# Ledicia/Molecular-Dynamics-Simulation---Lennard-Jones-monoatomic-fluid

Hardware: AMD Instinct MI355X
Metric: md_steps_per_sec_n262144_fp64 (higher is better)
Workload: dtype f64

## Files before the change

molecular-dynamics-simulation---lennard-jones-monoatomic-fluid_amd/csrc/ljmd_capi.cpp:

```cpp
#include "ljmd_engine.h"
#include "ljmd_multi.h"

#include <new>

namespace ljmdh {

int entry_checks(const ljmd_t *h, const char *who, unsigned checks)
{
    if ((checks & kHandle) && !h) return fail(nullptr, LJMD_ERR_INVALID_ARG, "%s: NULL handle", who);
    if ((checks & kHaveState) && !h->have_state) return fail(h, LJMD_ERR_STATE, "%s: no state has been set", who);
    if ((checks & kHaveAccel) && !h->have_accel)
        return fail(h, LJMD_ERR_STATE, "%s: accelerations not initialised (call ljmd_compute_forces first)", who);
    if ((checks & kNotPoisoned) && h->poisoned)
        return fail(h, LJMD_ERR_STATE, "%s: handle poisoned by an earlier failure; call ljmd_set_state", who);
    return LJMD_OK;
}

}

extern "C" {

const char *ljmd_version(void) { return "ljmd 0.6.0 gfx950"; }

int32_t ljmd_device_count(void)
// ... 61 lines not shown
                      int32_t n_gpus, const int32_t *devices)
{
    return ljmdm::create(out, n, box_length, dt, rc, precision_mode, n_gpus, devices);
}


int ljmd_set_state(ljmd_t *h, const double *rx, const double *ry, const double *rz,
                   const double *vx, const double *vy, const double *vz)
{
    LJMD_TRY(entry_checks(h, "ljmd_set_state", kHandle));
    if (!rx || !ry || !rz || !vx || !vy || !vz)
        return fail(h, LJMD_ERR_INVALID_ARG, "ljmd_set_state: NULL array");
    if (h->multi) return ljmdm::set_state(h, rx, ry, rz, vx, vy, vz);
    h->boxes_valid = false;
    h->drift_prefused = false;
    h->step_open = false;
    ljmdt::tcf_new_trajectory(&h->tcf);
    LJMD_HIP(h, hipSetDevice(h->device));
    if (h->poisoned) {
        LJMD_HIP(h, hipStreamSynchronize(h->stream));
        LJMD_HIP(h, hipMemcpy(&h->ring_issued, h->d_ring_pos, sizeof(unsigned), hipMemcpyDeviceToHost));
        h->ring_consumed = h->ring_issued;
        h->forces_pending = false;
        h->gather_done_for_step = false;
        h->fold_pending = false;
        h->poisoned = false;
    }
    const size_t S = h->plan.S, P = h->plan.P;
    double lo[3] = {INFINITY, INFINITY, INFINITY}, hi[3] = {-INFINITY, -INFINITY, -INFINITY};
    const double *src[3] = {rx, ry, rz};
    bool finite = true;
    for (int g = 0; g < h->G; ++g)
        for (int ax = 0; ax < 3; ++ax) {
            double *dst = h->h_stage + ((size_t)g * 3 + ax) * P;
            const double *s = src[ax] + (size_t)g * S;
// ... 123 lines not shown
{
    if (h->multi) return ljmdm::enqueue_steps(h, nsteps, sampled);
    static_assert(LJMD_MAX_PENDING_STEPS == kRingCap, "LJMD_MAX_PENDING_STEPS out of sync with the record ring");
    if (ring_guard && (h->ring_issued - h->ring_consumed) + (unsigned)nsteps > kRingCap)
        return fail(h, LJMD_ERR_STATE, "%s: %u + %d pending steps exceed LJMD_MAX_PENDING_STEPS", who,
                    h->ring_issued - h->ring_consumed, nsteps);
    LJMD_HIP(h, hipSetDevice(h->device));
    const bool keep = h->want_energy;
    for (int s = 0; s < nsteps; ++s) {
        EventSet *q = next_events(h);
        if (sampled) h->want_energy = s == nsteps - 1;
        int rc_ = enqueue_drift(h, q);
        if (rc_ == LJMD_OK) rc_ = enqueue_forces(h, true, q, s + 1 < nsteps);
        if (rc_ != LJMD_OK) {
            h->want_energy = keep;
            h->poisoned = true;
            return rc_;
        }
    }
    h->want_energy = keep;
    return LJMD_OK;
}

int collect_steps(ljmd_t *h, int32_t nsteps, double *epot, double *ekin, double *d_epot, double *dd_epot, const char *who)
{
    LJMD_TRY(entry_checks(h, who, kHandle));
    if (nsteps < 0 || nsteps > (int)kRingCap) return fail(h, LJMD_ERR_INVALID_ARG, "%s: nsteps out of range", who);
    LJMD_TRY(entry_checks(h, who, kNotPoisoned));
    if (h->multi) return ljmdm::collect_steps(h, nsteps, epot, ekin, d_epot, dd_epot);
    if (h->G != 1) return fail(h, LJMD_ERR_STATE, "%s: sharded engine; use ljmd_read_partials", who);
// ... 389 lines not shown
```

molecular-dynamics-simulation---lennard-jones-monoatomic-fluid_amd/csrc/ljmd_common.cpp:

```cpp
#include "ljmd_common.h"
#include "ljmd_internal.h"

#include <algorithm>
#include <cstdio>
#include <cstring>
#include <limits>

namespace ljmdh {

using namespace ljmdk;

thread_local std::string g_last_error = "";

int failv(std::string *handle_err, int code, const char *fmt, va_list ap)
{
    char buf[512];
    vsnprintf(buf, sizeof buf, fmt, ap);
    g_last_error = buf;
    if (handle_err) *handle_err = buf;
    return code;
}

int check_sim_params(const char *who, int n, double box_length, double dt, double rc)
{
// ... 50 lines not shown
        const char *v = std::getenv(name);
        if (v && *v) return std::atoi(v);
        return std::nullopt;
    };
    Knobs k;
    k.sort = flag("LJMD_SORT", k.sort);
    k.force_generic = flag("LJMD_FORCE_GENERIC", k.force_generic);
    k.force_collectives = flag("LJMD_FORCE_COLLECTIVES", k.force_collectives);
    k.fuse = flag("LJMD_FUSE", k.fuse);
    k.fuse_tail = flag("LJMD_FUSE_TAIL", k.fuse_tail);
    k.fuse_defer_record = flag("LJMD_FUSE_DEFER_RECORD", k.fuse_defer_record);
    k.xcd_remap = std::max(0, env_int("LJMD_N3_XCD_REMAP", k.xcd_remap));
    k.inject_failure_at_step = env_int("LJMD_INJECT_FAILURE_AT_STEP", k.inject_failure_at_step);
    k.exchange_alltoall = is("LJMD_FORCE_EXCHANGE", "alltoall");
    k.resort_every = opt_int("LJMD_RESORT_EVERY");
    k.n3_row_tiles = env_int("LJMD_N3_ROW_TILES", k.n3_row_tiles);
    k.n3_wg_waves = env_int("LJMD_N3_WG_WAVES", k.n3_wg_waves);
    k.slab_budget_gb = std::max(1, env_int("LJMD_SLAB_BUDGET_GB", k.slab_budget_gb));
    k.n3_both_ties = flag("LJMD_N3_BOTH_TIES", k.n3_both_ties);
    k.n3_min_n = env_int("LJMD_N3_MIN_N", k.n3_min_n);
    k.n3 = flag("LJMD_N3", k.n3);
    k.n3_target_waves = opt_int("LJMD_N3_TARGET_WAVES");
    k.n3_clusters = flag("LJMD_N3_CLUSTERS", k.n3_clusters);
    k.n3_pertile = flag("LJMD_N3_PERTILE", k.n3_pertile);
    k.reduce_split = opt_int("LJMD_REDUCE_SPLIT");
    if (k.reduce_split) k.reduce_split = std::max(0, *k.reduce_split);
    k.walk_chunk = opt_int("LJMD_WALK_CHUNK");
    k.fp32_far_stream = flag("LJMD_FP32_FAR_STREAM", k.fp32_far_stream);
    k.fp32_vfar = flag("LJMD_FP32_VFAR", k.fp32_vfar);
    {
// ... 87 lines not shown
```

molecular-dynamics-simulation---lennard-jones-monoatomic-fluid_amd/csrc/ljmd_common.h:

```cpp
#ifndef LJMD_COMMON_H
#define LJMD_COMMON_H

#include "ljmd.h"

#include <hip/hip_runtime.h>

#include <cstdarg>
#include <cstddef>
#include <cstdint>
#include <cstdlib>
#include <optional>
#include <string>

namespace ljmdh {

extern thread_local std::string g_last_error;

constexpr double kPi = 3.1415926535897932384626433832795;

int failv(std::string *handle_err, int code, const char *fmt, va_list ap);

inline int fail(std::nullptr_t, int code, const char *fmt, ...)
{
    va_list ap;
// ... 57 lines not shown

void scalars_from_exact_sums(const uint64_t (&ordered)[5][3], double te, double td, double tdd, bool have_e, bool have_k,
                             double *epot, double *ekin, double *d_epot, double *dd_epot);

struct Knobs {
    bool sort = true;
    bool force_generic = false;
    bool force_collectives = false;
    bool fuse = true;
    bool fuse_tail = true;
    bool fuse_defer_record = true;
    int xcd_remap = 4;
    int inject_failure_at_step = -1;
    bool exchange_alltoall = false;
    std::optional<int> resort_every;
    int n3_row_tiles = 0;
    int n3_wg_waves = 0;
    int slab_budget_gb = 64;
    bool n3_both_ties = true;
    int n3_min_n = 4096;
    bool n3 = true;
    std::optional<int> n3_target_waves;
    bool n3_clusters = true;
    bool n3_pertile = true;
    std::optional<int> reduce_split;
    std::optional<int> walk_chunk;
    bool fp32_far_stream = true;
    bool fp32_vfar = true;
    double fp32_split = 5.0;
    bool overlap_exchange = true;
// ... 11 lines not shown
```

molecular-dynamics-simulation---lennard-jones-monoatomic-fluid_amd/csrc/ljmd_engine.cpp:

```cpp
#include "ljmd_engine.h"

namespace ljmdh {

bool fast_path_ok(const ljmd_t *h) { return h->plan.rc_allows_fast && h->positions_compact && !h->knobs.force_generic; }

double *wg_part_now(ljmd_t *h) { return h->d_wg_part + (h->plan.fuse_tail ? (size_t)h->fold_parity * h->wg_part_stride : 0); }

PairArgs pair_args(ljmd_t *h, bool fast)
{
    PairArgs a;
    a.pos = h->d_pos;
    a.slab = h->d_slab;
    a.wg_part = wg_part_now(h);
    a.mask = h->d_mask;
    a.bbox = h->d_bbox;
    a.inline_mask = (fast && h->plan.fuse_tail && !h->plan.use_n3) ? 1 : 0;
    a.rc2_skin = h->rc2 * (1.0 + 1e-10);
    a.n = h->n;
    a.S = h->plan.S;
    a.P = h->plan.P;
    a.G = h->G;
    a.rank = h->rank;
    a.TB = h->plan.TB;
    a.T = h->plan.T;
// ... 133 lines not shown

EventSet *next_events(ljmd_t *h)
{
    if (!h->profiling || h->ev_used >= (size_t)kMaxProfiledLaunches) return nullptr;
    if (h->ev_used == h->ev_pool.size()) {
        EventSet q;
        for (auto &e : q.e)
            if (hipEventCreate(&e) != hipSuccess) return nullptr;
        h->ev_pool.push_back(q);
    }
    EventSet *q = &h->ev_pool[h->ev_used++];
    q->has_pos_x = q->has_force_x = false;
    return q;
}

int resort(ljmd_t *h, bool with_accel)
{
    {
    LJMD_HIP(h, launch_iota(h->d_idx, h->plan.P, h->stream));
    LJMD_HIP(h, hipMemcpyAsync(h->d_idx2, h->d_idx, (size_t)h->plan.P * sizeof(int), hipMemcpyDeviceToDevice,
                               h->stream));
    int *cur = h->d_idx, *nxt = h->d_idx2;
    for (size_t l = 0; l < h->plan.kd_level_nseg.size(); ++l) {
        const double *axis = own_block(h) + (size_t)h->kd_axis[l] * h->plan.P;
        LJMD_HIP(h, kd_level(h->d_cub, h->cub_bytes, axis, h->L, h->d_kd_keys, h->d_kd_keys2, cur, nxt, h->plan.S,
                             h->plan.kd_level_nseg[l], h->d_kd_offsets + h->plan.kd_level_off[l], h->stream));
        std::swap(cur, nxt);
    }
    if (cur != h->d_idx2)
        LJMD_HIP(h, hipMemcpyAsync(h->d_idx2, cur, (size_t)h->plan.P * sizeof(int), hipMemcpyDeviceToDevice,
                                   h->stream));
    }
    const size_t bytes3 = 3 * (size_t)h->plan.P * sizeof(double);
    double *sets[4] = {own_block(h), h->d_ru, h->d_v, h->d_a};
    for (int k = 0; k < (with_accel ? 4 : 3); ++k) {
        LJMD_HIP(h, launch_gather3(sets[k], h->d_tmp3, h->d_idx2, h->plan.P, h->stream));
        LJMD_HIP(h, hipMemcpyAsync(sets[k], h->d_tmp3, bytes3, hipMemcpyDeviceToDevice, h->stream));
    }
    LJMD_HIP(h, launch_gather_perm(h->d_perm, h->d_perm2, h->d_idx2, h->plan.P, h->stream));
    std::swap(h->d_perm, h->d_perm2);
    h->perm_dirty = true;
    h->steps_since_sort = 0;
    return LJMD_OK;
}

int refresh_perm(ljmd_t *h)
{
    if (!h->perm_dirty) return LJMD_OK;
    LJMD_HIP(h, hipMemcpyAsync(h->h_perm.data(), h->d_perm, (size_t)h->plan.P * sizeof(int), hipMemcpyDeviceToHost,
                               h->stream));
    LJMD_HIP(h, hipStreamSynchronize(h->stream));
    h->perm_dirty = false;
    return LJMD_OK;
}

bool use_comm_stream(const ljmd_t *h) { return h->knobs.overlap_exchange && h->comm_stream != nullptr; }

int comm_begin(ljmd_t *h)
// ... 65 lines not shown
                                          h->mode == LJMD_PRECISION_FP32_FORCE ? h->d_desc_far : nullptr, h->d_desc2, h->stream));
        else
            LJMD_HIP(h, launch_tile_mask(ga, h->stream));
        if (q) LJMD_HIP(h, hipEventRecord(q->e[2], h->stream));
        if (h->plan.use_n3) {
            const dim3 grid((h->plan.NGo + h->plan.wg_waves - 1) / h->plan.wg_waves, h->plan.nslab_n);
            N3Args na = n3_args(h);
            na.xcd_remap = (h->knobs.xcd_remap > 0 && (int)grid.x >= kXcdMinGroups && grid.x % (8 * h->knobs.xcd_remap) == 0) ? h->knobs.xcd_remap : 0;
            const bool far_beside = h->mode == LJMD_PRECISION_FP32_FORCE && h->far_stream != nullptr;
            split = h->plan.split_s1 > 0 && h->side_stream != nullptr;
            if (split) {
                const int s1 = h->plan.split_s1;
                LJMD_HIP(h, hipEventRecord(h->ev_side_go, h->stream));
                LJMD_HIP(h, hipStreamWaitEvent(h->side_stream, h->ev_side_go, 0));
                LJMD_HIP(h, launch_pair_n3(na, dim3(grid.x, s1), h->plan.wg_waves, h->stream));
                N3Args nb = na;
                nb.by0 = s1;
                LJMD_HIP(h, launch_pair_n3(nb, dim3(grid.x, grid.y - s1), h->plan.wg_waves, h->side_stream));
                LJMD_HIP(h, launch_reduce_forces_split(reduce_args(h, h->plan.nslab_n, true), 1, h->stream));
                LJMD_HIP(h, hipEventRecord(h->ev_side_done, h->side_stream));
                LJMD_HIP(h, hipStreamWaitEvent(h->stream, h->ev_side_done, 0));
            } else if (far_beside) {
                LJMD_HIP(h, hipEventRecord(h->ev_far_go, h->stream));
                LJMD_HIP(h, hipStreamWaitEvent(h->far_stream, h->ev_far_go, 0));
            } else {
                LJMD_HIP(h, launch_pair_n3(na, grid, h->plan.wg_waves, h->stream));
            }
            nslab = h->plan.nslab_n;
            n_wg = grid.x * grid.y * h->plan.wg_waves;
            n3 = true;
            if (h->mode == LJMD_PRECISION_FP32_FORCE) {
                const dim3 fgrid(h->plan.NGo, h->plan.nslab_n);
                N3Args fa = n3_args(h);
                fa.mask = h->d_mask_far;
                fa.slab_i = h->d_slab + (size_t)h->plan.nslab_n * 3 * h->plan.P;
                fa.slab_j = h->d_slab_j2;
// ... 163 lines not shown

int enqueue_drift_positions(ljmd_t *h, EventSet *q, bool *split)
{
    if (q) LJMD_HIP(h, hipEventRecord(q->e[0], h->stream));
    h->gather_done_for_step = false;
    const bool resort_now = h->plan.sort_enabled && fast_path_ok(h) && h->steps_since_sort + 1 >= h->plan.resort_every;
    *split = !resort_now;
    LJMD_HIP(h, launch_drift_kick(integrate_args(h), resort_now ? 0 : 1, h->stream));
    h->positions_compact = true;
    h->positions_wide = false;
    if (h->plan.sort_enabled && fast_path_ok(h) && ++h->steps_since_sort >= h->plan.resort_every) {
        if (*split) {
            LJMD_HIP(h, launch_drift_kick(integrate_args(h), 2, h->stream));
            *split = false;
        }
        return resort(h, false);
    }
    return LJMD_OK;
}

int enqueue_drift_velocities(ljmd_t *h)
{
    LJMD_HIP(h, launch_drift_kick(integrate_args(h), 2, h->stream));
    return LJMD_OK;
}

int enqueue_drift(ljmd_t *h, EventSet *q)
{
    const bool collectives = h->comm && (h->G > 1 || h->knobs.force_collectives);
    if (collectives && use_comm_stream(h)) {
        bool split = false;
// ... 11 lines not shown
        LJMD_HIP(h, hipEventRecord(h->ev_gather_done, h->comm_stream));
        rc_ = enqueue_drift_velocities(h);
        if (rc_ != LJMD_OK) return rc_;
        LJMD_HIP(h, hipStreamWaitEvent(h->stream, h->ev_gather_done, 0));
        h->gather_done_for_step = true;
        return LJMD_OK;
    }
    if (q) LJMD_HIP(h, hipEventRecord(q->e[0], h->stream));
    h->gather_done_for_step = false;
    const bool resort_now = h->plan.sort_enabled && fast_path_ok(h) && h->steps_since_sort + 1 >= h->plan.resort_every;
    if (h->drift_prefused) {
        h->drift_prefused = false;
        h->boxes_valid = !resort_now && fast_path_ok(h);
        h->positions_compact = true;
        h->positions_wide = false;
        if (h->plan.sort_enabled && fast_path_ok(h) && ++h->steps_since_sort >= h->plan.resort_every) return resort(h, false);
        return LJMD_OK;
    }
    IntegrateArgs ia = integrate_args(h);
    h->boxes_valid = h->knobs.fuse && h->G == 1 && h->n <= 65536 && !resort_now && fast_path_ok(h);
    if (h->boxes_valid) {
        ia.bbox = h->d_bbox;
        ia.pos_tc = h->plan.use_n3 ? h->d_pos_tc : nullptr;
    }
    LJMD_HIP(h, launch_drift_kick(ia, 0, h->stream));
    h->positions_compact = true;
    h->positions_wide = false;
    if (h->plan.sort_enabled && fast_path_ok(h) && ++h->steps_since_sort >= h->plan.resort_every)
        return resort(h, false);
    return LJMD_OK;
}

int fetch_ring(ljmd_t *h, unsigned count)
{
    if (count > h->ring_issued - h->ring_consumed)
        return fail(h, LJMD_ERR_STATE, "requested %u step records but only %u are pending", count,
                    h->ring_issued - h->ring_consumed);
    h->ring_consumed = h->ring_issued - count;
    unsigned done = 0;
    while (done < count) {
        const unsigned pos = (h->ring_consumed + done) % kRingCap;
        const unsigned run = std::min(count - done, kRingCap - pos);
        LJMD_HIP(h, hipMemcpyAsync(h->h_ring + (size_t)done * h->rec_stride,
                                   h->d_ring + (size_t)pos * h->rec_stride,
// ... 11 lines not shown
```

molecular-dynamics-simulation---lennard-jones-monoatomic-fluid_amd/csrc/ljmd_engine.h:

```cpp
#ifndef LJMD_ENGINE_H
#define LJMD_ENGINE_H

#include "ljmd_common.h"

#include <rccl/rccl.h>

#include <algorithm>
#include <cmath>
#include <cstdio>
#include <cstring>
#include <limits>
#include <mutex>
#include <vector>

#include "ljmd_internal.h"
#include "ljmd_resident.h"

using namespace ljmdk;

namespace ljmdh {

constexpr unsigned kRingCap = 4096;
constexpr int kTargetWorkgroups = 2048;
constexpr int kXcdMinGroups = 256;
constexpr int kMixedMinN = 16384;
constexpr long kN3ItemsFor4 = 6000;
constexpr long kN3ItemsFor2 = 1000;
constexpr long kN3LargeItems = 131072;
constexpr int kN3MidTargetItems = 32768;
constexpr int kBothTiesMaxGroups = 128;
constexpr int kFuseTailMaxRowTiles = 2;
constexpr int kFuseTailMaxN = 20000;
constexpr int kReduceSplitMinN = 131072;
constexpr int kReduceSplitShare = 8;
constexpr int kMaxProfiledLaunches = 4096;
constexpr int kEventsPerLaunch = 9;

struct EventSet {
    hipEvent_t e[kEventsPerLaunch];
    bool has_pos_x = false, has_force_x = false;
};

struct LaunchPlan {
    int S = 0, P = 0;
    int TB = 0, T = 0, W = 0;
    bool rc_allows_fast = false;
    bool sort_enabled = true;
    int resort_every = 20;
    std::vector<int> kd_level_nseg;
    std::vector<size_t> kd_level_off;
    std::vector<int> kd_offsets;
    int nslab_g = 1, chunk_g = 0;
    int nslab_t = 1, chunk_t = 0;
    bool use_n3 = false;
    int wg_waves = 1;
    bool both_ties = false;
    int uchunk = 0;
    int CS = 0, CS2 = 0, j_by_group = 0;
    int NG = 0, NGo = 0, Dmax = 0, nslab_n = 1, dchunk = 0;
    int rt = kRowTiles;
    bool fuse_tail = false;
    int split_s1 = 0, split_j1 = 0;
    int nslab_max = 1, n_wg_max = 0;
    int n_ke = 0;
};

int plan_engine(const SimParams &sim, int n, int n_ranks, int precision_mode, const Knobs &k, LaunchPlan *out);

}

struct ljmd_multi;

using namespace ljmdh;

struct ljmd : ljmdh::SimParams {
    ljmd_multi *multi = nullptr;
    bool poisoned = false;
// ... 48 lines not shown
    std::vector<int> kd_axis;
    int *d_kd_offsets = nullptr;
    unsigned long long *d_kd_keys = nullptr, *d_kd_keys2 = nullptr;

    unsigned ring_consumed = 0;
    unsigned ring_issued = 0;
    bool fold_pending = false;
    ljmdk::FinalizeArgs pending_fold{};
    int fold_parity = 0;
    size_t wg_part_stride = 0;
    double *d_slab_j = nullptr;
    unsigned char *d_flag_j = nullptr;
    double *d_red_part = nullptr;
    hipStream_t side_stream = nullptr;
    hipEvent_t ev_side_go = nullptr, ev_side_done = nullptr;
    uint64_t *d_mask_far = nullptr;
    double *d_slab_j2 = nullptr;
    unsigned char *d_flag_j2 = nullptr;
    double *d_fpart = nullptr, *d_frecv = nullptr;
    double *d_fall = nullptr;
    bool forces_pending = false;
    bool external_force_exchange = false;
    int pending_n_wg = 0;
    double pending_scale = 0.5;

    double *h_stage = nullptr;
    double *h_ring = nullptr;
    std::vector<int> h_perm;
    bool perm_dirty = false;

// ... 38 lines not shown

enum : unsigned { kHandle = 1, kHaveState = 2, kHaveAccel = 4, kNotPoisoned = 8 };
int entry_checks(const ljmd_t *h, const char *who, unsigned checks);

inline double *own_block(ljmd_t *h) { return h->d_pos + (size_t)h->rank * 3 * h->plan.P; }
inline bool needs_force_exchange(const ljmd_t *h) { return h->plan.use_n3 && (h->G > 1 || h->knobs.force_collectives); }
bool fast_path_ok(const ljmd_t *h);
IntegrateArgs integrate_args(ljmd_t *h);

int allocate_engine(ljmd_t *h);
void release(ljmd_t *h);
void release_resident(ljmd_t *h);
int download_state(ljmd_t *h, double *const dsts[12], unsigned n_records);
int upload_shard3(ljmd_t *h, double *dst, const double *x, const double *y, const double *z);
int resort(ljmd_t *h, bool with_accel);
int refresh_perm(ljmd_t *h);
bool use_comm_stream(const ljmd_t *h);
int comm_begin(ljmd_t *h);
int comm_end(ljmd_t *h);
int allgather_on(ljmd_t *h, hipStream_t s);

int enqueue_drift(ljmd_t *h, EventSet *q);
int enqueue_drift_positions(ljmd_t *h, EventSet *q, bool *split);
int enqueue_drift_velocities(ljmd_t *h);
int enqueue_pair_forces(ljmd_t *h, EventSet *q);
int enqueue_kick(ljmd_t *h, bool kick, EventSet *q);
int enqueue_forces(ljmd_t *h, bool kick, EventSet *q, bool next_drift = false);
int fetch_ring(ljmd_t *h, unsigned count);
void combine_one(const ljmd_t *h, const double *recs, int n_ranks, double *epot, double *ekin, double *d_epot,
                 double *dd_epot);
// ... 15 lines not shown
```

molecular-dynamics-simulation---lennard-jones-monoatomic-fluid_amd/csrc/ljmd_internal.h:

```cpp
#ifndef LJMD_INTERNAL_H
#define LJMD_INTERNAL_H

#include <hip/hip_runtime.h>
#include <stdint.h>

namespace ljmdk {

constexpr int kBlock = 256;
constexpr int kWavesPerBlock = kBlock / 64;
constexpr int kTile = 64;
#ifndef LJMD_ROW_TILES
#define LJMD_ROW_TILES 4
#endif
constexpr int kRowTiles = LJMD_ROW_TILES;
constexpr unsigned kAllRows = (1u << kRowTiles) - 1u;
constexpr int kSlotAlign = (kRowTiles * 64 > 256) ? kRowTiles * 64 : 256;
constexpr int kPartialStride = 8;
constexpr int kFoldBlocks = 128;
constexpr int kDirectFoldMax = 20480;
constexpr int kBoxStride = 8;

struct PairArgs {
    const double *pos;
    double *slab;
// ... 220 lines not shown
hipError_t launch_pair_fixed(const FixedArgs &a, dim3 grid, hipStream_t s);
hipError_t launch_fixed_tail(const FixedTailArgs &a, bool kick, bool energy, bool ke_only, hipStream_t s);
hipError_t launch_fixed_fold(const FixedFoldArgs &a, hipStream_t s);
hipError_t launch_rdf_histogram(const RdfArgs &a, dim3 grid, hipStream_t s);
hipError_t launch_time_origin(const TimeOriginArgs &a, bool vacf, int n_origins, hipStream_t s);
hipError_t launch_tile_boxes(const GeometryArgs &a, hipStream_t s);
hipError_t launch_tile_mask(const GeometryArgs &a, hipStream_t s);
hipError_t launch_tile_class(const GeometryArgs &a, double invL, double rc2, int S, int NGo, unsigned *desc,
                             unsigned *desc_far, float *desc2 , hipStream_t s);

size_t kd_temp_bytes(int count);
hipError_t launch_iota(int *idx, int P, hipStream_t s);
hipError_t kd_level(void *temp, size_t temp_bytes, const double *coord_axis, double L, unsigned long long *keys,
                    unsigned long long *keys_out, int *idx, int *idx_out, int S, int nseg, const int *seg_offsets,
                    hipStream_t s);
constexpr int kMigrateRows = 10;
hipError_t launch_iota_blocked(int *idx, int n, int S, int P, hipStream_t s);
hipError_t launch_iota_offset(int *idx, int count, int P, int offset, hipStream_t s);
hipError_t kd_level_blocked(void *temp, size_t temp_bytes, const double *pos, int axis, int P, double L,
                            unsigned long long *keys, unsigned long long *keys_out, int *idx, int *idx_out, int n, int nseg,
                            const int *seg_offsets, hipStream_t s);
hipError_t launch_migrate_pack(const double *ru, const double *v, const double *a, const int *perm, const int *gid0,
                               double *block, int S, int P, hipStream_t s);
hipError_t launch_migrate_select(const double *pos_all, const double *mig_all, const int *mine, double *new_pos, double *ru,
                                 double *v, double *a, int *gid0, int S, int P, hipStream_t s);
hipError_t launch_gather3(const double *src, double *dst, const int *idx, int P, hipStream_t s);
hipError_t launch_gather_perm(const int *src, int *dst, const int *idx, int P, hipStream_t s);


__device__ __forceinline__ double wave_sum(double v)
// ... 170 lines not shown
```

molecular-dynamics-simulation---lennard-jones-monoatomic-fluid_amd/csrc/ljmd_plan.cpp:

```cpp
#include "ljmd_engine.h"

namespace ljmdh {

namespace {
int rt_align(int uchunk, int rt)
{
    int m = 1;
    while ((m * uchunk) % rt != 0) ++m;
    return m;
}
}

int plan_engine(const SimParams &sim, int n, int n_ranks, int precision_mode, const Knobs &k, LaunchPlan *out)
{
    LaunchPlan p;
    p.S = n / n_ranks;
    p.P = ((p.S + kSlotAlign - 1) / kSlotAlign) * kSlotAlign;
    p.TB = p.P / kTile;
    p.T = n_ranks * p.TB;
    p.W = (p.T + 63) / 64;
    p.rc_allows_fast = sim.rc <= (1.0 - 1e-9) * 0.5 * sim.L;
    p.sort_enabled = k.sort && n >= 1024;
    p.resort_every = std::max(1, k.resort_every.value_or(n >= 1000000 ? 5 : n >= 131072 ? 10 : n > 40000 ? 20
                                                              : n > kFuseTailMaxN ? 50 : 200));
// ... 3 lines not shown
        while (true) {
            bool any = false;
            for (size_t j = 0; j + 1 < bounds.size(); ++j) any = any || (bounds[j + 1] - bounds[j] > 1);
            if (!any) break;
            p.kd_level_off.push_back(p.kd_offsets.size());
            p.kd_level_nseg.push_back((int)bounds.size() - 1);
            for (int b : bounds) p.kd_offsets.push_back(std::min(b * kTile, p.S));
            std::vector<int> next;
            for (size_t j = 0; j + 1 < bounds.size(); ++j) {
                next.push_back(bounds[j]);
                const int t = bounds[j + 1] - bounds[j];
                if (t > 1) next.push_back(bounds[j] + (t + 1) / 2);
            }
            next.push_back(tiles);
            bounds.swap(next);
        }
    }

    const int row_blocks = p.P / kBlock;
    {
        int ns = (kTargetWorkgroups + row_blocks - 1) / row_blocks;
        ns = std::max(1, std::min(ns, (n + 63) / 64));
        p.chunk_g = ((n + ns - 1) / ns + 7) / 8 * 8;
        p.nslab_g = (n + p.chunk_g - 1) / p.chunk_g;
    }
    {
        int ns = (kTargetWorkgroups + row_blocks - 1) / row_blocks;
        ns = std::max(1, std::min(ns, p.T));
        p.chunk_t = (p.T + ns - 1) / ns;
        p.nslab_t = (p.T + p.chunk_t - 1) / p.chunk_t;
// ... 40 lines not shown
            p.uchunk = (n_units + nsu - 1) / nsu;
        }
        p.nslab_n = (n_units + p.uchunk - 1) / p.uchunk;
    }
    p.fuse_tail = k.fuse && k.fuse_tail && n_ranks == 1 && n <= kFuseTailMaxN && p.rc_allows_fast &&
                  precision_mode == LJMD_PRECISION_FP64 && (!p.use_n3 || (p.rt <= kFuseTailMaxRowTiles && p.wg_waves == 1));
    if (n_ranks == 1 && precision_mode == LJMD_PRECISION_FP64 && p.use_n3 && p.rc_allows_fast && !p.fuse_tail &&
        p.rt == kRowTiles && p.wg_waves == 1 && !p.j_by_group && !k.force_collectives) {
        const int S = p.nslab_n;
        const int m = rt_align(p.uchunk, p.rt);
        const int deferred = k.reduce_split.value_or(n >= kReduceSplitMinN ? (S + kReduceSplitShare - 1) / kReduceSplitShare : 0);
        if (deferred >= 1 && m < S) {
            const int s1 = std::max(m, (std::max(0, S - deferred) / m) * m);
            p.split_s1 = s1;
            p.split_j1 = s1 * p.uchunk / p.rt;
        }
    }
    const bool mixed = precision_mode == LJMD_PRECISION_FP32_FORCE;
    if (mixed && (!p.use_n3 || n < kMixedMinN))
        return fail(nullptr, LJMD_ERR_INVALID_ARG,
                    "ljmd_create: LJMD_PRECISION_FP32_FORCE needs the Newton-3 path and n >= %d", kMixedMinN);
    p.nslab_max = std::max(std::max(p.nslab_g, p.nslab_t), p.use_n3 ? p.nslab_n * (mixed ? 2 : 1) : 1);
    p.n_wg_max = std::max(row_blocks * std::max(p.nslab_g, p.nslab_t),
                          (p.NGo + 4) * p.nslab_n * (mixed ? 2 : 1));
    p.n_ke = row_blocks;
    *out = std::move(p);
    return LJMD_OK;
}

}
// ... 1 lines not shown
```

molecular-dynamics-simulation---lennard-jones-monoatomic-fluid_amd/csrc/ljmd_sort.hip:

```cpp
#include <hip/hip_runtime.h>
#include <hipcub/hipcub.hpp>

#include "ljmd_internal.h"

namespace ljmdk {

__global__ __launch_bounds__(kBlock) void gather3_kernel(const double *src, double *dst, const int *idx, int P)
{
    const int i = blockIdx.x * kBlock + threadIdx.x;
    if (i >= P) return;
    const int s = idx[i];
    dst[i] = src[s];
    dst[P + i] = src[P + s];
    dst[2 * (size_t)P + i] = src[2 * (size_t)P + s];
}

__global__ __launch_bounds__(kBlock) void gather_perm_kernel(const int *src, int *dst, const int *idx, int P)
{
    const int i = blockIdx.x * kBlock + threadIdx.x;
    if (i < P) dst[i] = src[idx[i]];
}

constexpr int kCoordBits = 24;

// ... 35 lines not shown

hipError_t kd_level(void *temp, size_t temp_bytes, const double *coord_axis, double L, unsigned long long *keys,
                    unsigned long long *keys_out, int *idx, int *idx_out, int S, int nseg, const int *seg_offsets,
                    hipStream_t s)
{
    hipLaunchKernelGGL(kd_keys_kernel, dim3((S + kBlock - 1) / kBlock), dim3(kBlock), 0, s, coord_axis, idx, keys,
                       seg_offsets, nseg, S, (double)(1u << kCoordBits) / L);
    hipError_t e = hipGetLastError();
    if (e != hipSuccess) return e;
    int segbits = 1;
    while ((1 << segbits) < nseg) ++segbits;
    return hipcub::DeviceRadixSort::SortPairs(temp, temp_bytes, keys, keys_out, idx, idx_out, S, 0,
                                              kCoordBits + segbits, s);
}

__global__ __launch_bounds__(kBlock) void iota_blocked_kernel(int *idx, int n, int S, int P)
{
    const int k = blockIdx.x * kBlock + threadIdx.x;
    if (k < n) idx[k] = (k / S) * P + k % S;
}

__global__ __launch_bounds__(kBlock) void kd_keys_blocked_kernel(const double *pos, int axis, int P, const int *idx,
                                                                 unsigned long long *keys, const int *seg_offsets, int nseg,
                                                                 int n, double scale)
{
    const int i = blockIdx.x * kBlock + threadIdx.x;
    if (i >= n) return;
    int lo = 0, hi = nseg;
    while (hi - lo > 1) {
        const int mid = (lo + hi) >> 1;
// ... 114 lines not shown
```

molecular-dynamics-simulation---lennard-jones-monoatomic-fluid_amd/csrc/ljmd_storage.cpp:

```cpp
#include "ljmd_engine.h"

namespace ljmdh {

int allocate_engine(ljmd_t *h)
{
    const bool mixed = h->mode == LJMD_PRECISION_FP32_FORCE;
    const std::vector<int> &kd = h->plan.kd_offsets;
    LJMD_HIP(h, hipSetDevice(h->device));
    LJMD_HIP(h, hipStreamCreateWithFlags(&h->stream, hipStreamNonBlocking));
    const size_t P3 = 3 * (size_t)h->plan.P * sizeof(double);
    LJMD_HIP(h, hipMalloc(&h->d_pos, P3 * h->G));
    LJMD_HIP(h, hipMalloc(&h->d_ru, P3));
    LJMD_HIP(h, hipMalloc(&h->d_v, P3));
    LJMD_HIP(h, hipMalloc(&h->d_a, P3));
    LJMD_HIP(h, hipMalloc(&h->d_tmp3, P3));
    LJMD_HIP(h, hipMalloc(&h->d_slab, P3 * h->plan.nslab_max));
    h->wg_part_stride = 2 * (size_t)h->plan.n_wg_max;
    LJMD_HIP(h, hipMalloc(&h->d_wg_part, (h->plan.fuse_tail ? 2 : 1) * h->wg_part_stride * sizeof(double)));
    if (h->plan.use_n3) {
        const size_t n_blk = (size_t)h->plan.T * h->plan.CS;
        LJMD_HIP(h, hipMalloc(&h->d_slab_j, n_blk * 3 * kTile * sizeof(double)));
        LJMD_HIP(h, hipMalloc(&h->d_flag_j, n_blk));
        LJMD_HIP(h, hipMemsetAsync(h->d_flag_j, 0, n_blk, h->stream));
        LJMD_HIP(h, hipMalloc(&h->d_desc, (size_t)h->plan.NGo * h->plan.T * sizeof(unsigned)));
        if (h->plan.rt == kRowTiles && h->plan.wg_waves == 1 && h->knobs.n3_clusters)
            LJMD_HIP(h, hipMalloc(&h->d_desc2, (size_t)h->plan.NGo * h->plan.T * 8 * sizeof(float)));
        LJMD_HIP(h, hipMalloc(&h->d_pos_tc, P3 * h->G));
    }
    if (h->plan.split_s1 > 0) {
        LJMD_HIP(h, hipMalloc(&h->d_red_part, (size_t)h->plan.TB * kWavesPerBlock * 3 * kTile * sizeof(double)));
        int least = 0, greatest = 0;
        LJMD_HIP(h, hipDeviceGetStreamPriorityRange(&least, &greatest));
        LJMD_HIP(h, hipStreamCreateWithPriority(&h->side_stream, hipStreamNonBlocking, least));
        LJMD_HIP(h, hipEventCreateWithFlags(&h->ev_side_go, hipEventDisableTiming));
        LJMD_HIP(h, hipEventCreateWithFlags(&h->ev_side_done, hipEventDisableTiming));
    }
    if (mixed && h->knobs.fp32_far_stream) {
        LJMD_HIP(h, hipStreamCreateWithFlags(&h->far_stream, hipStreamNonBlocking));
        LJMD_HIP(h, hipEventCreateWithFlags(&h->ev_far_go, hipEventDisableTiming));
        LJMD_HIP(h, hipEventCreateWithFlags(&h->ev_far_done, hipEventDisableTiming));
    }
    if (mixed) {
        LJMD_HIP(h, hipMalloc(&h->d_mask_far, (size_t)h->plan.TB * h->plan.W * sizeof(uint64_t)));
        LJMD_HIP(h, hipMalloc(&h->d_desc_far, (size_t)h->plan.NGo * h->plan.T * sizeof(unsigned)));
        const size_t n_blk2 = (size_t)h->plan.T * h->plan.CS2;
        LJMD_HIP(h, hipMalloc(&h->d_slab_j2, n_blk2 * 3 * kTile * sizeof(float)));
        LJMD_HIP(h, hipMalloc(&h->d_flag_j2, n_blk2));
        LJMD_HIP(h, hipMemsetAsync(h->d_flag_j2, 0, n_blk2, h->stream));
    }
    LJMD_HIP(h, hipMalloc(&h->d_fpart, P3 * (needs_force_exchange(h) ? h->G : 1)));
// ... 43 lines not shown
}

void release(ljmd_t *h)
{
    if (!h) return;
    if (h->device >= 0) (void)hipSetDevice(h->device);
    if (h->stream) (void)hipStreamSynchronize(h->stream);
    release_resident(h);
    if (h->comm_stream) (void)hipStreamSynchronize(h->comm_stream);
    if (h->comm) (void)ncclCommDestroy(h->comm);
    if (h->comm_stream) (void)hipStreamDestroy(h->comm_stream);
    if (h->far_stream) {
        (void)hipStreamSynchronize(h->far_stream);
        (void)hipStreamDestroy(h->far_stream);
    }
    if (h->side_stream) {
        (void)hipStreamSynchronize(h->side_stream);
        (void)hipStreamDestroy(h->side_stream);
    }
    if (h->ev_side_go) (void)hipEventDestroy(h->ev_side_go);
    if (h->ev_side_done) (void)hipEventDestroy(h->ev_side_done);
    if (h->ev_far_go) (void)hipEventDestroy(h->ev_far_go);
    if (h->ev_far_done) (void)hipEventDestroy(h->ev_far_done);
    if (h->ev_pos_ready) (void)hipEventDestroy(h->ev_pos_ready);
    if (h->ev_gather_done) (void)hipEventDestroy(h->ev_gather_done);
    for (auto &q : h->ev_pool)
        for (auto &e : q.e) (void)hipEventDestroy(e);
    void *dev[] = {h->d_pos, h->d_ru, h->d_v, h->d_a, h->d_slab, h->d_wg_part, h->d_ke_part, h->d_ring,
                   h->d_ring_pos, h->d_bbox, h->d_mask, h->d_idx, h->d_idx2,
                   h->d_perm, h->d_perm2, h->d_tmp3, h->d_cub, h->d_slab_j, h->d_flag_j, h->d_fpart, h->d_frecv, h->d_fall,
// ... 88 lines not shown
```

Measured before the change: 55.88.

## Fuse deep kd-sort levels into one shared-memory kernel and optionally overlap sort

```diff
diff --git a/molecular-dynamics-simulation---lennard-jones-monoatomic-fluid_amd/csrc/ljmd_capi.cpp b/molecular-dynamics-simulation---lennard-jones-monoatomic-fluid_amd/csrc/ljmd_capi.cpp
--- a/molecular-dynamics-simulation---lennard-jones-monoatomic-fluid_amd/csrc/ljmd_capi.cpp
+++ b/molecular-dynamics-simulation---lennard-jones-monoatomic-fluid_amd/csrc/ljmd_capi.cpp
@@ -99,11 +99,13 @@
     if (h->multi) return ljmdm::set_state(h, rx, ry, rz, vx, vy, vz);
     h->boxes_valid = false;
     h->drift_prefused = false;
+    h->order_pending = false;
     h->step_open = false;
     ljmdt::tcf_new_trajectory(&h->tcf);
     LJMD_HIP(h, hipSetDevice(h->device));
     if (h->poisoned) {
         LJMD_HIP(h, hipStreamSynchronize(h->stream));
+        if (h->sort_stream) LJMD_HIP(h, hipStreamSynchronize(h->sort_stream));
         LJMD_HIP(h, hipMemcpy(&h->ring_issued, h->d_ring_pos, sizeof(unsigned), hipMemcpyDeviceToHost));
         h->ring_consumed = h->ring_issued;
         h->forces_pending = false;
@@ -257,6 +259,7 @@
         if (rc_ == LJMD_OK) rc_ = enqueue_forces(h, true, q, s + 1 < nsteps);
         if (rc_ != LJMD_OK) {
             h->want_energy = keep;
+            h->order_pending = false;
             h->poisoned = true;
             return rc_;
         }
diff --git a/molecular-dynamics-simulation---lennard-jones-monoatomic-fluid_amd/csrc/ljmd_common.cpp b/molecular-dynamics-simulation---lennard-jones-monoatomic-fluid_amd/csrc/ljmd_common.cpp
--- a/molecular-dynamics-simulation---lennard-jones-monoatomic-fluid_amd/csrc/ljmd_common.cpp
+++ b/molecular-dynamics-simulation---lennard-jones-monoatomic-fluid_amd/csrc/ljmd_common.cpp
@@ -88,6 +88,8 @@
     k.inject_failure_at_step = env_int("LJMD_INJECT_FAILURE_AT_STEP", k.inject_failure_at_step);
     k.exchange_alltoall = is("LJMD_FORCE_EXCHANGE", "alltoall");
     k.resort_every = opt_int("LJMD_RESORT_EVERY");
+    k.sort_fused = std::max(0, env_int("LJMD_SORT_FUSED", k.sort_fused));
+    k.sort_lag = flag("LJMD_SORT_LAG", k.sort_lag);
     k.n3_row_tiles = env_int("LJMD_N3_ROW_TILES", k.n3_row_tiles);
     k.n3_wg_waves = env_int("LJMD_N3_WG_WAVES", k.n3_wg_waves);
     k.slab_budget_gb = std::max(1, env_int("LJMD_SLAB_BUDGET_GB", k.slab_budget_gb));
diff --git a/molecular-dynamics-simulation---lennard-jones-monoatomic-fluid_amd/csrc/ljmd_common.h b/molecular-dynamics-simulation---lennard-jones-monoatomic-fluid_amd/csrc/ljmd_common.h
--- a/molecular-dynamics-simulation---lennard-jones-monoatomic-fluid_amd/csrc/ljmd_common.h
+++ b/molecular-dynamics-simulation---lennard-jones-monoatomic-fluid_amd/csrc/ljmd_common.h
@@ -95,6 +95,8 @@
     int inject_failure_at_step = -1;
     bool exchange_alltoall = false;
     std::optional<int> resort_every;
+    int sort_fused = 1;
+    bool sort_lag = false;
     int n3_row_tiles = 0;
     int n3_wg_waves = 0;
     int slab_budget_gb = 64;
diff --git a/molecular-dynamics-simulation---lennard-jones-monoatomic-fluid_amd/csrc/ljmd_engine.cpp b/molecular-dynamics-simulation---lennard-jones-monoatomic-fluid_amd/csrc/ljmd_engine.cpp
--- a/molecular-dynamics-simulation---lennard-jones-monoatomic-fluid_amd/csrc/ljmd_engine.cpp
+++ b/molecular-dynamics-simulation---lennard-jones-monoatomic-fluid_amd/csrc/ljmd_engine.cpp
@@ -171,23 +171,60 @@
     return q;
 }
 
+}
+
+namespace ljmdk {
+__attribute__((weak)) hipError_t launch_kd_fused(const KdFusedArgs &, hipStream_t) { return hipErrorNotSupported; }
+}
+
+namespace ljmdh {
+
 int resort(ljmd_t *h, bool with_accel)
 {
-    {
-    LJMD_HIP(h, launch_iota(h->d_idx, h->plan.P, h->stream));
+    h->order_pending = false;
+    const int rc_ = sort_order(h, h->stream);
+    return rc_ == LJMD_OK ? apply_order(h, with_accel) : rc_;
+}
+
+int sort_order(ljmd_t *h, hipStream_t s)
+{
+    LJMD_HIP(h, launch_iota(h->d_idx, h->plan.P, s));
     LJMD_HIP(h, hipMemcpyAsync(h->d_idx2, h->d_idx, (size_t)h->plan.P * sizeof(int), hipMemcpyDeviceToDevice,
-                               h->stream));
+                               s));
     int *cur = h->d_idx, *nxt = h->d_idx2;
-    for (size_t l = 0; l < h->plan.kd_level_nseg.size(); ++l) {
+    const int n_levels = (int)h->plan.kd_level_nseg.size(), fused_from = h->plan.kd_fused_from;
+    for (int l = 0; l < fused_from; ++l) {
         const double *axis = own_block(h) + (size_t)h->kd_axis[l] * h->plan.P;
         LJMD_HIP(h, kd_level(h->d_cub, h->cub_bytes, axis, h->L, h->d_kd_keys, h->d_kd_keys2, cur, nxt, h->plan.S,
-                             h->plan.kd_level_nseg[l], h->d_kd_offsets + h->plan.kd_level_off[l], h->stream));
+                             h->plan.kd_level_nseg[l], h->d_kd_offsets + h->plan.kd_level_off[l], s));
         std::swap(cur, nxt);
     }
+    if (fused_from < n_levels) {
+        KdFusedArgs fa{};
+        fa.pos = own_block(h);
+        fa.idx = cur;
+        fa.idx_out = nxt;
+        fa.offsets = h->d_kd_offsets;
+        fa.L = h->L;
+        fa.P = h->plan.P;
+        fa.cap = h->plan.kd_fused_cap;
+        fa.n_levels = n_levels - fused_from;
+        fa.n_roots = h->plan.kd_level_nseg[fused_from];
+        for (int l = fused_from; l < n_levels; ++l) {
+            fa.level_off[l - fused_from] = (int)h->plan.kd_level_off[l];
+            fa.level_nseg[l - fused_from] = h->plan.kd_level_nseg[l];
+            fa.axis[l - fused_from] = h->kd_axis[l];
+        }
+        LJMD_HIP(h, launch_kd_fused(fa, s));
+        std::swap(cur, nxt);
+    }
     if (cur != h->d_idx2)
-        LJMD_HIP(h, hipMemcpyAsync(h->d_idx2, cur, (size_t)h->plan.P * sizeof(int), hipMemcpyDeviceToDevice,
-                                   h->stream));
-    }
+        LJMD_HIP(h, hipMemcpyAsync(h->d_idx2, cur, (size_t)h->plan.P * sizeof(int), hipMemcpyDeviceToDevice, s));
+    return LJMD_OK;
+}
+
+int apply_order(ljmd_t *h, bool with_accel)
+{
     const size_t bytes3 = 3 * (size_t)h->plan.P * sizeof(double);
     double *sets[4] = {own_block(h), h->d_ru, h->d_v, h->d_a};
     for (int k = 0; k < (with_accel ? 4 : 3); ++k) {
@@ -199,6 +236,13 @@
     h->perm_dirty = true;
     h->steps_since_sort = 0;
     return LJMD_OK;
+}
+
+int resort_in_step(ljmd_t *h)
+{
+    if (!h->order_pending) return resort(h, false);
+    h->order_pending = false;
+    return apply_order(h, false);
 }
 
 int refresh_perm(ljmd_t *h)
@@ -294,12 +338,24 @@
                 LJMD_HIP(h, hipEventRecord(h->ev_side_go, h->stream));
                 LJMD_HIP(h, hipStreamWaitEvent(h->side_stream, h->ev_side_go, 0));
                 LJMD_HIP(h, launch_pair_n3(na, dim3(grid.x, s1), h->plan.wg_waves, h->stream));
+                const bool sort_ahead = h->plan.sort_lag && (h->kick_hint == 1 || h->step_open) && !h->order_pending &&
+                                        h->steps_since_sort + 1 >= h->plan.resort_every;
+                if (sort_ahead) {
+                    LJMD_HIP(h, hipStreamWaitEvent(h->sort_stream, h->ev_side_go, 0));
+                    const int rc_ = sort_order(h, h->sort_stream);
+                    if (rc_ != LJMD_OK) return rc_;
+                    LJMD_HIP(h, hipEventRecord(h->ev_sort_done, h->sort_stream));
+                }
                 N3Args nb = na;
                 nb.by0 = s1;
                 LJMD_HIP(h, launch_pair_n3(nb, dim3(grid.x, grid.y - s1), h->plan.wg_waves, h->side_stream));
                 LJMD_HIP(h, launch_reduce_forces_split(reduce_args(h, h->plan.nslab_n, true), 1, h->stream));
                 LJMD_HIP(h, hipEventRecord(h->ev_side_done, h->side_stream));
                 LJMD_HIP(h, hipStreamWaitEvent(h->stream, h->ev_side_done, 0));
+                if (sort_ahead) {
+                    LJMD_HIP(h, hipStreamWaitEvent(h->stream, h->ev_sort_done, 0));
+                    h->order_pending = true;
+                }
             } else if (far_beside) {
                 LJMD_HIP(h, hipEventRecord(h->ev_far_go, h->stream));
                 LJMD_HIP(h, hipStreamWaitEvent(h->far_stream, h->ev_far_go, 0));
@@ -493,7 +549,7 @@
             LJMD_HIP(h, launch_drift_kick(integrate_args(h), 2, h->stream));
             *split = false;
         }
-        return resort(h, false);
+        return resort_in_step(h);
     }
     return LJMD_OK;
 }
@@ -535,7 +591,7 @@
         h->boxes_valid = !resort_now && fast_path_ok(h);
         h->positions_compact = true;
         h->positions_wide = false;
-        if (h->plan.sort_enabled && fast_path_ok(h) && ++h->steps_since_sort >= h->plan.resort_every) return resort(h, false);
+        if (h->plan.sort_enabled && fast_path_ok(h) && ++h->steps_since_sort >= h->plan.resort_every) return resort_in_step(h);
         return LJMD_OK;
     }
     IntegrateArgs ia = integrate_args(h);
@@ -548,7 +604,7 @@
     h->positions_compact = true;
     h->positions_wide = false;
     if (h->plan.sort_enabled && fast_path_ok(h) && ++h->steps_since_sort >= h->plan.resort_every)
-        return resort(h, false);
+        return resort_in_step(h);
     return LJMD_OK;
 }
 
diff --git a/molecular-dynamics-simulation---lennard-jones-monoatomic-fluid_amd/csrc/ljmd_engine.h b/molecular-dynamics-simulation---lennard-jones-monoatomic-fluid_amd/csrc/ljmd_engine.h
--- a/molecular-dynamics-simulation---lennard-jones-monoatomic-fluid_amd/csrc/ljmd_engine.h
+++ b/molecular-dynamics-simulation---lennard-jones-monoatomic-fluid_amd/csrc/ljmd_engine.h
@@ -31,6 +31,7 @@
 constexpr int kBothTiesMaxGroups = 128;
 constexpr int kFuseTailMaxRowTiles = 2;
 constexpr int kFuseTailMaxN = 20000;
+constexpr int kKdFusedCap = 1024;
 constexpr int kReduceSplitMinN = 131072;
 constexpr int kReduceSplitShare = 8;
 constexpr int kMaxProfiledLaunches = 4096;
@@ -50,6 +51,8 @@
     std::vector<int> kd_level_nseg;
     std::vector<size_t> kd_level_off;
     std::vector<int> kd_offsets;
+    int kd_fused_from = 0;
+    int kd_fused_cap = 0;
     int nslab_g = 1, chunk_g = 0;
     int nslab_t = 1, chunk_t = 0;
     bool use_n3 = false;
@@ -61,6 +64,7 @@
     int rt = kRowTiles;
     bool fuse_tail = false;
     int split_s1 = 0, split_j1 = 0;
+    bool sort_lag = false;
     int nslab_max = 1, n_wg_max = 0;
     int n_ke = 0;
 };
@@ -139,6 +143,9 @@
     double *d_red_part = nullptr;
     hipStream_t side_stream = nullptr;
     hipEvent_t ev_side_go = nullptr, ev_side_done = nullptr;
+    bool order_pending = false;
+    hipStream_t sort_stream = nullptr;
+    hipEvent_t ev_sort_done = nullptr;
     uint64_t *d_mask_far = nullptr;
     double *d_slab_j2 = nullptr;
     unsigned char *d_flag_j2 = nullptr;
@@ -207,6 +214,8 @@
 int download_state(ljmd_t *h, double *const dsts[12], unsigned n_records);
 int upload_shard3(ljmd_t *h, double *dst, const double *x, const double *y, const double *z);
 int resort(ljmd_t *h, bool with_accel);
+int sort_order(ljmd_t *h, hipStream_t s);
+int apply_order(ljmd_t *h, bool with_accel);
 int refresh_perm(ljmd_t *h);
 bool use_comm_stream(const ljmd_t *h);
 int comm_begin(ljmd_t *h);
diff --git a/molecular-dynamics-simulation---lennard-jones-monoatomic-fluid_amd/csrc/ljmd_internal.h b/molecular-dynamics-simulation---lennard-jones-monoatomic-fluid_amd/csrc/ljmd_internal.h
--- a/molecular-dynamics-simulation---lennard-jones-monoatomic-fluid_amd/csrc/ljmd_internal.h
+++ b/molecular-dynamics-simulation---lennard-jones-monoatomic-fluid_amd/csrc/ljmd_internal.h
@@ -258,6 +258,22 @@
 hipError_t kd_level(void *temp, size_t temp_bytes, const double *coord_axis, double L, unsigned long long *keys,
                     unsigned long long *keys_out, int *idx, int *idx_out, int S, int nseg, const int *seg_offsets,
                     hipStream_t s);
+constexpr int kKdFusedMaxLevels = 8;
+struct KdFusedArgs {
+    const double *pos;
+    const int *idx;
+    int *idx_out;
+    const int *offsets;
+    double L;
+    int P;
+    int cap;
+    int n_levels;
+    int n_roots;
+    int level_off[kKdFusedMaxLevels];
+    int level_nseg[kKdFusedMaxLevels];
+    int axis[kKdFusedMaxLevels];
+};
+hipError_t launch_kd_fused(const KdFusedArgs &a, hipStream_t s);
 constexpr int kMigrateRows = 10;
 hipError_t launch_iota_blocked(int *idx, int n, int S, int P, hipStream_t s);
 hipError_t launch_iota_offset(int *idx, int count, int P, int offset, hipStream_t s);
diff --git a/molecular-dynamics-simulation---lennard-jones-monoatomic-fluid_amd/csrc/ljmd_plan.cpp b/molecular-dynamics-simulation---lennard-jones-monoatomic-fluid_amd/csrc/ljmd_plan.cpp
--- a/molecular-dynamics-simulation---lennard-jones-monoatomic-fluid_amd/csrc/ljmd_plan.cpp
+++ b/molecular-dynamics-simulation---lennard-jones-monoatomic-fluid_amd/csrc/ljmd_plan.cpp
@@ -41,6 +41,15 @@
             }
             next.push_back(tiles);
             bounds.swap(next);
+        }
+        const int n_levels = (int)p.kd_level_nseg.size();
+        p.kd_fused_from = n_levels;
+        p.kd_fused_cap = (k.sort_fused == 1024 || k.sort_fused == 2048 || k.sort_fused == 4096) ? k.sort_fused : kKdFusedCap;
+        for (int l = 0; l < n_levels && k.sort_fused != 0 && p.kd_fused_from == n_levels; ++l) {
+            const int *off = p.kd_offsets.data() + p.kd_level_off[l];
+            int widest = 0;
+            for (int j = 0; j < p.kd_level_nseg[l]; ++j) widest = std::max(widest, off[j + 1] - off[j]);
+            if (widest <= p.kd_fused_cap && n_levels - l <= kKdFusedMaxLevels) p.kd_fused_from = l;
         }
     }
 
@@ -111,6 +120,7 @@
             const int s1 = std::max(m, (std::max(0, S - deferred) / m) * m);
             p.split_s1 = s1;
             p.split_j1 = s1 * p.uchunk / p.rt;
+            p.sort_lag = k.sort_lag && p.sort_enabled && p.resort_every >= 2;
         }
     }
     const bool mixed = precision_mode == LJMD_PRECISION_FP32_FORCE;
diff --git a/molecular-dynamics-simulation---lennard-jones-monoatomic-fluid_amd/csrc/ljmd_sort.hip b/molecular-dynamics-simulation---lennard-jones-monoatomic-fluid_amd/csrc/ljmd_sort.hip
--- a/molecular-dynamics-simulation---lennard-jones-monoatomic-fluid_amd/csrc/ljmd_sort.hip
+++ b/molecular-dynamics-simulation---lennard-jones-monoatomic-fluid_amd/csrc/ljmd_sort.hip
@@ -73,6 +73,77 @@
                                               kCoordBits + segbits, s);
 }
 
+template <int CAP>
+__global__ __launch_bounds__(CAP / 4) void kd_fused_kernel(KdFusedArgs a)
+{
+    __shared__ int s_idx[2][CAP];
+    __shared__ unsigned long long s_key[CAP];
+    const int *root = a.offsets + a.level_off[0];
+    const int base = root[blockIdx.x];
+    const int m = min(root[blockIdx.x + 1] - base, CAP);
+    const int p0 = 4 * (int)threadIdx.x;
+    const double scale = (double)(1u << kCoordBits) / a.L;
+#pragma unroll
+    for (int e = 0; e < 4; ++e)
+        if (p0 + e < m) s_idx[0][p0 + e] = a.idx[base + p0 + e];
+    __syncthreads();
+    int cur = 0;
+    for (int l = 0; l < a.n_levels; ++l) {
+        const int *seg_offsets = a.offsets + a.level_off[l];
+        const int nseg = a.level_nseg[l];
+        const double *coord = a.pos + (size_t)a.axis[l] * a.P;
+        unsigned long long mine[4] = {0, 0, 0, 0};
+        int id[4] = {0, 0, 0, 0};
+        int first = m, last = 0;
+#pragma unroll
+        for (int e = 0; e < 4; ++e) {
+            const int p = p0 + e;
+            if (p >= m) continue;
+            const int i = base + p;
+            int lo = 0, hi = nseg;
+            while (hi - lo > 1) {
+                const int mid = (lo + hi) >> 1;
+                if (seg_offsets[mid] <= i) lo = mid; else hi = mid;
+            }
+            id[e] = s_idx[cur][p];
+            const double x = coord[id[e]] * scale;
+            const unsigned long long q = (unsigned long long)fmin(fmax(x, 0.0), (double)((1u << kCoordBits) - 1));
+            mine[e] = ((unsigned long long)lo << (kCoordBits + 12)) | (q << 12) | (unsigned long long)p;
+            s_key[p] = mine[e];
+            first = min(first, max(seg_offsets[lo] - base, 0));
+            last = max(last, min(seg_offsets[lo + 1] - base, m));
+        }
+        __syncthreads();
+        int cnt[4] = {0, 0, 0, 0};
+        for (int j = first; j < last; ++j) {
+            const unsigned long long k = s_key[j];
+#pragma unroll
+            for (int e = 0; e < 4; ++e) cnt[e] += k < mine[e] ? 1 : 0;
+        }
+#pragma unroll
+        for (int e = 0; e < 4; ++e)
+            if (p0 + e < m) s_idx[cur ^ 1][first + cnt[e]] = id[e];
+        __syncthreads();
+        cur ^= 1;
+    }
+#pragma unroll
+    for (int e = 0; e < 4; ++e)
+        if (p0 + e < m) a.idx_out[base + p0 + e] = s_idx[cur][p0 + e];
+}
+
+hipError_t launch_kd_fused(const KdFusedArgs &a, hipStream_t s)
+{
+    if (a.cap == 4096)
+        hipLaunchKernelGGL(kd_fused_kernel<4096>, dim3(a.n_roots), dim3(1024), 0, s, a);
+    else if (a.cap == 2048)
+        hipLaunchKernelGGL(kd_fused_kernel<2048>, dim3(a.n_roots), dim3(512), 0, s, a);
+    else if (a.cap == 1024)
+        hipLaunchKernelGGL(kd_fused_kernel<1024>, dim3(a.n_roots), dim3(256), 0, s, a);
+    else
+        return hipErrorInvalidValue;
+    return hipGetLastError();
+}
+
 __global__ __launch_bounds__(kBlock) void iota_blocked_kernel(int *idx, int n, int S, int P)
 {
     const int k = blockIdx.x * kBlock + threadIdx.x;
diff --git a/molecular-dynamics-simulation---lennard-jones-monoatomic-fluid_amd/csrc/ljmd_storage.cpp b/molecular-dynamics-simulation---lennard-jones-monoatomic-fluid_amd/csrc/ljmd_storage.cpp
--- a/molecular-dynamics-simulation---lennard-jones-monoatomic-fluid_amd/csrc/ljmd_storage.cpp
+++ b/molecular-dynamics-simulation---lennard-jones-monoatomic-fluid_amd/csrc/ljmd_storage.cpp
@@ -34,6 +34,10 @@
         LJMD_HIP(h, hipStreamCreateWithPriority(&h->side_stream, hipStreamNonBlocking, least));
         LJMD_HIP(h, hipEventCreateWithFlags(&h->ev_side_go, hipEventDisableTiming));
         LJMD_HIP(h, hipEventCreateWithFlags(&h->ev_side_done, hipEventDisableTiming));
+        if (h->plan.sort_lag) {
+            LJMD_HIP(h, hipStreamCreateWithPriority(&h->sort_stream, hipStreamNonBlocking, least));
+            LJMD_HIP(h, hipEventCreateWithFlags(&h->ev_sort_done, hipEventDisableTiming));
+        }
     }
     if (mixed && h->knobs.fp32_far_stream) {
         LJMD_HIP(h, hipStreamCreateWithFlags(&h->far_stream, hipStreamNonBlocking));
@@ -107,6 +111,11 @@
         (void)hipStreamSynchronize(h->far_stream);
         (void)hipStreamDestroy(h->far_stream);
     }
+    if (h->sort_stream) {
+        (void)hipStreamSynchronize(h->sort_stream);
+        (void)hipStreamDestroy(h->sort_stream);
+    }
+    if (h->ev_sort_done) (void)hipEventDestroy(h->ev_sort_done);
     if (h->side_stream) {
         (void)hipStreamSynchronize(h->side_stream);
         (void)hipStreamDestroy(h->side_stream);
```

New measurement: 55.89, median of 2. About the same (+0.0%).
